# Julia-Tempering/Pigeons.jl

Hardware: AMD Instinct MI355X
Metric: replica-steps/sec (explore+swap), toy_mvn d=1024, n_chains=1024; round-trip rate (higher is better)
Workload: dtype f64

## Files before the change

### pigeons.jl_amd/csrc/pte_slice8.hpp

```cpp
#pragma once
#include "pte_slice7.hpp"

namespace pte {

#ifndef PTE_S8_BD
#define PTE_S8_BD 3
#endif
#ifndef PTE_S8_BS
#define PTE_S8_BS 9
#endif
constexpr int S8_BD = PTE_S8_BD;

#ifndef PTE_S8_WAVES
#define PTE_S8_WAVES 4
#endif
template <int NLU, int S8_BS, int WINDOW, int DBL_MODE>
__device__ __forceinline__ void slice8_body(EngineDev e, SliceParams sp, const int64_t cl) {
    using namespace s7;
    constexpr int WIN = WINDOW, REFILL_AT = WINDOW - PTE_S7_MARGIN;
    constexpr bool FAST = (DBL_MODE == 2);
    static_assert(CAP_ITERS >= S8_BS, "lane 0 must be able to run past the speculative budget");
#ifndef PTE_S8_BLK
#define PTE_S8_BLK 256
#endif
    constexpr int BLK = PTE_S8_BLK, CPB = BLK / 64;
    constexpr bool HOLD_POLICY = (WIN == 512);
    __shared__ struct {
        double u[WIN];
        double e[WIN];
        double x[BLK];
        double we[256];
        unsigned long long ke[256];
        unsigned policy[HOLD_POLICY ? 2 : 0];
        double rex[HOLD_POLICY ? 64 : 0];
        unsigned rmeta[HOLD_POLICY ? 64 : 0];
    } sm;
    double (&s_u)[WIN] = sm.u; double (&s_e)[WIN] = sm.e; double (&s_x)[BLK] = sm.x; double (&s_we)[256] = sm.we; unsigned long long (&s_ke)[256] = sm.ke;
    const int lane = lane_id();
#ifdef PTE_PROFILE_WAVES
    const uint64_t wave_t0 = __builtin_amdgcn_s_memrealtime();
#endif
    for (int i = lane; i < 256; i += 64) { s_we[i] = ZIG_WE[i]; s_ke[i] = ZIG_KE[i]; }
    if constexpr (HOLD_POLICY) sm.policy[0] = g_rng_policy;
    const auto exp_seq = [&](SeqRng &rs) __attribute__((always_inline)) -> double {
        if constexpr (HOLD_POLICY)
            return randexp_from_raw_hot(rs, rs.next(), [&]() __attribute__((always_inline)) -> unsigned {
                return (unsigned)__builtin_amdgcn_readfirstlane((int)*(const volatile __attribute__((address_space(3))) unsigned *)&sm.policy[0]); });
        else
            return randexp_seq(rs);
    };
    __syncthreads();
    if (cl >= e.K) return;
    const int64_t c = e.c0 + cl;
    const int slot = e.slot_of_chain[cl];
    if (is_ref_chain(e, c)) {
        iid_refresh_recorded<NLU>(e, cl, c, slot, e.sd[c], lane);
        return;
    }
    const double lp_before = lp_before_explore(e, c, slot);
    const int64_t d = e.d;
    double *xrow = e.x + (int64_t)slot * e.ld;
    const int B = (int)((d + 63) >> 6);
    const double nhp = e.nhp[c];
    const double inv_nhp = 1.0 / nhp;
    const double inv_abs_nhp = -inv_nhp * (1.0 + 1e-6);
    const double w = sp.w;
    const double w11 = 1.1 * sp.w;
    const int cap_iters = min(sp.max_iter, CAP_ITERS);
    const int kcap = min(sp.p, 20);
    const bool shr_more = S8_BS < cap_iters;
    constexpr bool HAND_SHRINK = (S8_BS == PTE_S8_BS && S8_BS >= 6 && S8_BS <= 10);
    constexpr bool N_IS_KN = (DBL_MODE == 2) && HAND_SHRINK;

    const int hg = s7_level(lane);
    const int hrel = s7_pick(LO, hg, 0) + lane - s7_pick(BASE, hg, 0);

    const int succ_lo = s7_pick(LO, hg + 1, 0), succ_wd = s7_pick(WD, hg + 1, 0), succ_base = s7_pick(BASE, hg + 1, 0);
    const int succ_off = hrel - succ_lo;
    const int word_c = 0x10000 - succ_off;
    const int word_c9 = (1 << 20) - succ_off * 512;
    const uint64_t seed_in = e.rng[2 * slot];

    double BS = 0.0;
    for (int b = 0; b < B; ++b) {
        int64_t i = 64 * (int64_t)b + lane;
        double v = (i < d) ? xrow[i] : 0.0;
        double s = wave_sum_dpp(v * v);
        if (lane == b) BS = s;
    }
    double S = upper_tree_root<NLU>(BS);
    if (nhp * S == -INFINITY) { if (lane == 0) set_error(e, ERR_SLICE_SUPPORT, (int)c, -1); return; }

    uint64_t wseed = e.rng[2 * slot];
    const uint64_t gamma = e.rng[2 * slot + 1];
    int p = 0;
    uint64_t gamma_inv = gamma;
    for (int k = 0; k < 5; ++k) gamma_inv *= 2ull - gamma * gamma_inv;
    double wsum = 0.0;
    typedef unsigned mask2_t __attribute__((ext_vector_type(2)));
    typedef unsigned slow_mask_t __attribute__((ext_vector_type(WIN / 32)));
    typedef double draws8_t __attribute__((ext_vector_type(8)));
    typedef double draws2_t __attribute__((ext_vector_type(2)));
    slow_mask_t slow_w;
#ifdef PTE_PROFILE_SECTIONS
    long long prof[21] = {0, 0, 0, 0, 0, 0, 0, 0, 0, 0, 0, 0, 0, 0, 0, 0, 0, 0, 0, 0, 0};
#endif
    constexpr unsigned S8_UNRESOLVED = 0xFFFFu;
    auto fill_window = [&]() __attribute__((always_inline)) {
        __syncthreads();
        double acc = 0.0;
        double pend_x = 0.0;
        int pend_m = WIN;
#pragma unroll
        for (int k = 0; k < WIN / 64; ++k) {
            const int i = 64 * k + lane;
            const uint64_t r = mix64(wseed + (uint64_t)(i + 1) * gamma);
            const uint64_t ri = r & MASK52;
            const int idx = (int)(ri & 0xFF);
            const bool fast = ri < s_ke[idx];
            const double ev = (double)ri * s_we[idx];
            s_u[i] = u52_to_unit(r);
            s_e[i] = fast ? ev : __longlong_as_double(0x7ff8000000000000LL);
            acc += fast ? ev : 0.0;
            const uint64_t sb = ballot64(!fast);
            slow_w[2 * k] = (unsigned)sb; slow_w[2 * k + 1] = (unsigned)(sb >> 32);
            if constexpr (HOLD_POLICY) { pend_x = fast ? pend_x : ev; pend_m = fast ? pend_m : (i | (idx << 16)); }
        }
        wsum = wave_sum_dpp(acc);
        p = 0;
        __syncthreads();
        if constexpr (HOLD_POLICY) {
            __builtin_amdgcn_sched_barrier(0);
            const int pi = pend_m & 0xFFFF, pidx = pend_m >> 16;
            const double f1 = ZIG_FE[pidx], f0 = ZIG_FE[(pidx - 1) & 0xFF];
            const double un = s_u[min(pi + 1, WIN - 1)], en = s_e[min(pi + 2, WIN - 1)];
            const double ex = exp(-pend_x);
            const bool in_reach = (pidx != 0) && (pi + 2 < WIN);
            const bool wedge = (f0 - f1) * un + f1 < ex;
            const unsigned used = !in_reach ? 0u : wedge ? 2u : (en == en) ? 3u : 0u;
            sm.rex[lane] = wedge ? pend_x : en;
            sm.rmeta[lane] = used ? ((unsigned)pi | (used << 16)) : S8_UNRESOLVED;
#ifdef PTE_PROFILE_SECTIONS
            prof[20] += (long long)__popcll(ballot64(used != 0u)) << 24;
#endif
            __syncthreads();
        }
    };
    fill_window();

    int dbl_z0 = 0, dbl_z1 = 0, dbl_one_hi = 0x3ff00000;
    if constexpr (DBL_MODE == 2) asm volatile("" : "+v"(dbl_z0), "+v"(dbl_z1), "+v"(dbl_one_hi));

    long long steps_sum = 0, fb_draws = 0, ex_total = 0;
    int steps_n = 0, acc_sum = 0, acc_n = 0, n_fb = 0;
    int err = 0, err_coord = -1;

    for (int pass = 0; pass < sp.n_passes && !err; ++pass) {
        for (int b = 0; BLK * (int64_t)b < d && !err; ++b) {
            const int64_t base = BLK * (int64_t)b;
            const int nl = (int)min((int64_t)BLK, d - base);
#pragma unroll
            for (int k = 0; k < CPB; ++k) s_x[64 * k + lane] = (64 * k + lane < nl) ? xrow[base + 64 * k + lane] : 0.0;
            __builtin_amdgcn_wave_barrier();
            double Sest = S * (1.0 + 1e-6) + wsum * inv_abs_nhp;
            int l = 0, l_end = nl;
            do {
                PROF_T(t0);
                if (__builtin_expect(p > REFILL_AT, 0)) { PROF_T(tr0); wseed += (uint64_t)p * gamma; fill_window(); Sest = Sest * (1.0 + 1e-6) + wsum * inv_abs_nhp; PROF_T(tr1); PROF_ADD(16, tr1 - tr0); PROF_ADD(17, 1); }
                const bool active = (l + hg) < nl;
                const double xold = s_x[(l + hg) & (BLK - 1)];
                int idx0 = p + hrel;
                double E = s_e[idx0];
                double u0 = s_u[idx0 + 1];
                double Vd[S8_BD];
#pragma unroll
                for (int it = 0; it < S8_BD; ++it) Vd[it] = s_u[idx0 + 2 + it];
                int ua = 0;
                if constexpr (DBL_MODE == 2) ua = (int)(uintptr_t)(const __attribute__((address_space(3))) double *)&s_u[idx0];
                int ex0 = 0;
                int cnt_base = 2;
                asm volatile("" : "+v"(cnt_base));
                if constexpr (DBL_MODE == 2) asm volatile("" : "+s"(ex0));
                unsigned slow_b;
                if constexpr (WIN == 512)
                    asm("s_lshr_b32 m0, %[p], 5\n" "s_nop 0\n" "s_movrels_b32 %[o], s84\n" "s_lshr_b32 %[o], %[o], %[p]"
                        : [o] "=&s"(slow_b) : [p] "s"(p), "{s[84:99]}"(slow_w) : "m0", "scc");
                else
                    asm("s_lshr_b32 m0, %[p], 5\n" "s_nop 0\n" "s_movrels_b32 %[o], s84\n" "s_lshr_b32 %[o], %[o], %[p]"
                        : [o] "=&s"(slow_b) : [p] "s"(p), "{s[84:91]}"(slow_w) : "m0", "scc");
                static_assert(WIN == 512 || WIN == 256, "the slow-path mask is sixteen or eight dwords");
                if (__builtin_expect((slow_b & 1u) != 0u, 0)) {
                    PROF_T(ts0);
                    if constexpr (HOLD_POLICY) {
                        const auto head_moves = [&](const double Ex, const int used) __attribute__((always_inline)) {
                            ex0 = used - 1;
                            if (lane == 0) { E = Ex; idx0 += ex0; cnt_base = 2 + ex0; ua += 8 * ex0; }
                            Sest += Ex * inv_abs_nhp;
                            ex_total += ex0;
                            u0 = s_u[idx0 + 1];
#pragma unroll
                            for (int it = 0; it < S8_BD; ++it) Vd[it] = s_u[idx0 + 2 + it];
                        };
                        const unsigned rmeta = (unsigned)__builtin_amdgcn_readfirstlane((int)sm.rmeta[p & 63]);
                        const double rex = sm.rex[p & 63];
                        if ((rmeta & 0xFFFFu) == (unsigned)p) {
                            head_moves(rex, (int)(rmeta >> 16));
#ifdef PTE_PROFILE_SECTIONS
                            asm volatile("" :: "v"(E), "v"(u0), "v"(Vd[S8_BD - 1]), "v"(Sest));
#endif
                            PROF_T(ts1); PROF_ADD(2, ts1 - ts0); PROF_ADD(20, 1);
                        } else {
                            SeqRng rs{wseed + (uint64_t)p * gamma, gamma};
                            const double Ex = exp_seq(rs);
                            const int used = (int)((rs.seed - (wseed + (uint64_t)p * gamma)) * gamma_inv);
                            if (used <= 17) head_moves(Ex, used);
#ifdef PTE_PROFILE_SECTIONS
                            asm volatile("" :: "v"(E), "v"(u0), "v"(Vd[S8_BD - 1]), "v"(Sest));
#endif
                            PROF_T(ts1); PROF_ADD(18, ts1 - ts0); PROF_ADD(19, 1);
                        }
                    } else {
                    SeqRng rs{wseed + (uint64_t)p * gamma, gamma};
                    const double Ex = exp_seq(rs);
                    const int used = (int)((rs.seed - (wseed + (uint64_t)p * gamma)) * gamma_inv);
                    if (used <= 17) {
                        ex0 = used - 1;
                        if (lane == 0) { E = Ex; idx0 += ex0; cnt_base = 2 + ex0; ua += 8 * ex0; }
                        Sest += Ex * inv_abs_nhp;
                        ex_total += ex0;
                        u0 = s_u[idx0 + 1];
#pragma unroll
                        for (int it = 0; it < S8_BD; ++it) Vd[it] = s_u[idx0 + 2 + it];
                    }
#ifdef PTE_PROFILE_SECTIONS
                    asm volatile("" :: "v"(E), "v"(u0), "v"(Vd[S8_BD - 1]), "v"(Sest));
#endif
                    PROF_T(ts1); PROF_ADD(18, ts1 - ts0); PROF_ADD(19, 1);
                    }
                }
                const double Enh = E * inv_nhp;
                const double Q = __builtin_fma(xold, xold, -Enh);
                const double Bq = Sest + fabs(Q);
                double dmin = fabs(Enh);
                auto test = [&](double v) __attribute__((always_inline)) -> double {
                    const double d = __builtin_fma(v, v, -Q);
                    dmin = fmin(dmin, fabs(d));
                    return d;
                };
                double LL = xold - w * u0;
                double RR = LL + w;
                double dL = test(LL), dR = test(RR);
                int kd = 0;
                double dmin_lr = 0.0;
                unsigned need_l0 = 0u;
                uint64_t need_m = 0ull;
                double thr2 = 0.0, mthr = 0.0, W = 0.0;
                int n = 0;
                uint64_t act_m = 0ull;
                draws8_t ud8 = 0.0; draws2_t ud2 = 0.0;
#if PTE_S8_BD >= 1 && PTE_S8_BD <= 4 && !defined(PTE_S8_DOUBLING_SELECTS)
                if constexpr (DBL_MODE == 2) {
                    double t_, wd_;
                    int sLh_, sRh_;
                    uint64_t sv_, sx_;
                    mask2_t sd_;
#define PTE_S8_CSTEP(V) \
                    "v_cmp_ge_f64 vcc, 0.5, " V "\n" \
                    "v_min_f64 v[102:103], v[114:115], v[116:117]\n" \
                    "v_cmpx_gt_f64_e64 %[sx], 0, v[102:103]\n" \
                    "v_add_f64 v[112:113], v[98:99], -v[96:97]\n" \
                    "v_add_u32 %[kd], 1, %[kd]\n" \
                    "v_add_u32 %[ua], 8, %[ua]\n" \
                    "v_cndmask_b32 v119, 0, %[one], vcc\n" \
                    "v_cndmask_b32 v121, %[one], v118, vcc\n" \
                    "v_fma_f64 v[96:97], -v[118:119], v[112:113], v[96:97]\n" \
                    "v_fma_f64 v[98:99], v[120:121], v[112:113], v[98:99]\n" \
                    "v_fma_f64 v[114:115], v[96:97], v[96:97], -v[110:111]\n" \
                    "v_fma_f64 v[116:117], v[98:99], v[98:99], -v[110:111]\n"
#define PTE_S8_CFOLD \
                    "v_min_f64 v[104:105], v[104:105], |v[114:115]|\n" \
                    "v_min_f64 v[104:105], v[104:105], |v[116:117]|\n"
#if PTE_S8_BS == 6
#define PTE_S8_UREADS_TAIL
#elif PTE_S8_BS == 7
#define PTE_S8_UREADS_TAIL "ds_read_b64 v[136:137], %[ua] offset:64\n"
#elif PTE_S8_BS == 8
#define PTE_S8_UREADS_TAIL "ds_read2_b64 v[136:139], %[ua] offset0:8 offset1:9\n"
#elif PTE_S8_BS == 9
#define PTE_S8_UREADS_TAIL "ds_read2_b64 v[136:139], %[ua] offset0:8 offset1:9\n" "ds_read_b64 v[140:141], %[ua] offset:80\n"
#else
#define PTE_S8_UREADS_TAIL "ds_read2_b64 v[136:139], %[ua] offset0:8 offset1:9\n" "ds_read2_b64 v[140:143], %[ua] offset0:10 offset1:11\n"
#endif
                    asm volatile("s_mov_b64 %[sv], exec\n"
#if PTE_S8_BD >= 2
                                 PTE_S8_CSTEP("%[V0]") PTE_S8_CFOLD
#endif
#if PTE_S8_BD >= 3
                                 PTE_S8_CSTEP("%[V1]") PTE_S8_CFOLD
#endif
#if PTE_S8_BD >= 4
                                 PTE_S8_CSTEP("%[V2]") PTE_S8_CFOLD
#endif
                                 PTE_S8_CSTEP("%[VL]")
                                 "s_mov_b64 exec, %[sv]\n"
                                 "ds_read2_b64 v[124:127], %[ua] offset0:2 offset1:3\n"
                                 "ds_read2_b64 v[128:131], %[ua] offset0:4 offset1:5\n"
                                 "ds_read2_b64 v[132:135], %[ua] offset0:6 offset1:7\n"
                                 PTE_S8_UREADS_TAIL
                                 "v_min_f64 v[102:103], v[114:115], v[116:117]\n"
                                 "v_cmp_gt_f64_e64 %[sd], 0, v[102:103]\n"
                                 PTE_S8_CFOLD
                                 "v_add_f64 %[mthr], %[Sest], |v[110:111]|\n"
                                 "v_max_f64 %[thr], |v[96:97]|, |v[98:99]|\n"
                                 "v_cmp_gt_i32_e64 %[act], %[nl], %[lg]\n"
                                 "v_add3_u32 v106, %[cb], %[so], %[kd]\n"
                                 "v_mul_f64 %[mthr], %[mthr], %[c_m]\n"
                                 "v_mul_f64 %[thr], %[thr], %[c_t]\n"
                                 "v_add_f64 v[112:113], v[98:99], -v[96:97]\n"
                                 : "+{v[96:97]}"(LL), "+{v[98:99]}"(RR), "+{v[114:115]}"(dL), "+{v[116:117]}"(dR), "+{v[104:105]}"(dmin), [kd] "+v"(kd), [ua] "+v"(ua),
                                   "=&{v[102:103]}"(t_), "=&{v[112:113]}"(wd_), "=&{v119}"(sLh_), "=&{v121}"(sRh_), [sv] "=&s"(sv_), [sx] "=&s"(sx_), [sd] "=&s"(sd_),
                                   "=&{v[124:139]}"(ud8), "=&{v[140:143]}"(ud2), [mthr] "=&v"(mthr), [thr] "=&v"(thr2), "=&{v106}"(n), [act] "=&s"(act_m)
                                 : "{v[110:111]}"(Q), "{v118}"(dbl_z0), "{v120}"(dbl_z1), [one] "v"(dbl_one_hi),
                                   [V0] "v"(Vd[0]), [V1] "v"(Vd[S8_BD > 2 ? 1 : 0]), [V2] "v"(Vd[S8_BD > 3 ? 2 : 0]), [VL] "v"(Vd[S8_BD - 1]),
                                   [Sest] "v"(Sest), [nl] "s"(nl), [lg] "v"(l + hg), [cb] "v"(cnt_base), [so] "v"(succ_off), [c_m] "s"(2e-12), [c_t] "s"(1e-6)
                                 : "vcc", "scc");
#undef PTE_S8_CSTEP
#undef PTE_S8_CFOLD
#undef PTE_S8_UREADS_TAIL
                    dmin_lr = t_; W = wd_;
                    need_m = (uint64_t)sd_.x | ((uint64_t)sd_.y << 32); need_l0 = __builtin_amdgcn_readfirstlane(sd_.x);
                } else
                if (DBL_MODE == 1 && sp.p >= S8_BD) {
                    double t_, wd_;
                    uint64_t sv_, sv2_;
#define PTE_S8_DSTEP(V) \
                    "v_min_f64 %[t], %[dL], %[dR]\n" \
                    "v_cmp_gt_f64 vcc, 0, %[t]\n" \
                    "s_and_saveexec_b64 %[sv], vcc\n" \
                    "v_add_u32 %[kd], 1, %[kd]\n" \
                    "v_add_f64 %[wd], %[RR], -%[LL]\n" \
                    "v_cmp_ge_f64 vcc, 0.5, " V "\n" \
                    "s_and_saveexec_b64 %[sv2], vcc\n" \
                    "v_add_f64 %[LL], %[LL], -%[wd]\n" \
                    "v_fma_f64 %[dL], %[LL], %[LL], -%[Q]\n" \
                    "v_min_f64 %[dmin], %[dmin], |%[dL]|\n" \
                    "s_andn2_b64 exec, %[sv2], exec\n" \
                    "v_add_f64 %[RR], %[RR], %[wd]\n" \
                    "v_fma_f64 %[dR], %[RR], %[RR], -%[Q]\n" \
                    "v_min_f64 %[dmin], %[dmin], |%[dR]|\n" \
                    "s_mov_b64 exec, %[sv]\n"
                    asm volatile(PTE_S8_DSTEP("%[V0]")
#if PTE_S8_BD >= 2
                                 PTE_S8_DSTEP("%[V1]")
#endif
#if PTE_S8_BD >= 3
                                 PTE_S8_DSTEP("%[V2]")
#endif
#if PTE_S8_BD >= 4
                                 PTE_S8_DSTEP("%[V3]")
#endif
                                 : [LL] "+v"(LL), [RR] "+v"(RR), [dL] "+v"(dL), [dR] "+v"(dR), [dmin] "+v"(dmin), [kd] "+v"(kd),
                                   [t] "=&v"(t_), [wd] "=&v"(wd_), [sv] "=&s"(sv_), [sv2] "=&s"(sv2_)
                                 : [Q] "v"(Q), [V0] "v"(Vd[0]), [V1] "v"(Vd[S8_BD > 1 ? 1 : 0]), [V2] "v"(Vd[S8_BD > 2 ? 2 : 0]), [V3] "v"(Vd[S8_BD > 3 ? 3 : 0])
                                 : "vcc", "scc");
#undef PTE_S8_DSTEP
                } else
#endif
#pragma unroll
                for (int it = 0; it < S8_BD; ++it) {
                    const bool need = (fmin(dL, dR) < 0.0) && it < sp.p;
                    const double V = Vd[it];
                    kd += need ? 1 : 0;
                    const bool left = V <= 0.5;
                    const double wd = RR - LL;
                    if constexpr (DBL_MODE == 0) {
                        const double sL = (need && left) ? 1.0 : 0.0, sR = (need && !left) ? 1.0 : 0.0;
                        LL = __builtin_fma(-sL, wd, LL);
                        RR = __builtin_fma(sR, wd, RR);
                        dL = __builtin_fma(LL, LL, -Q);
                        dR = __builtin_fma(RR, RR, -Q);
                        dmin = fmin(dmin, fmin(fabs(dL), fabs(dR)));
                    } else {
                        const double cand = left ? (LL - wd) : (RR + wd);
                        const double dc = __builtin_fma(cand, cand, -Q);
                        dmin = need ? fmin(dmin, fabs(dc)) : dmin;
                        const bool nl_ = need && left, nr_ = need && !left;
                        LL = nl_ ? cand : LL;
                        RR = nr_ ? cand : RR;
                        dL = nl_ ? dc : dL;
                        dR = nr_ ? dc : dR;
                    }
                }
#if !(PTE_S8_BD >= 1 && PTE_S8_BD <= 4) || defined(PTE_S8_DOUBLING_SELECTS)
                static_assert(DBL_MODE != 2, "PTE_S8_DBL_MODE == 2 needs the v_cmpx doubling block: 1 <= PTE_S8_BD <= 4 and no PTE_S8_DOUBLING_SELECTS");
#endif
                if constexpr (DBL_MODE != 2) dmin_lr = fmin(dL, dR);
                unsigned more_dbl;
                if constexpr (FAST) more_dbl = need_l0 & 1u;
                else more_dbl = ballot64(lane == 0 && (dmin_lr < 0.0) && kd < kcap) != 0ull ? 1u : 0u;
                if (__builtin_expect(more_dbl != 0u, 0)) {
                    bool need = (lane == 0);
                    while (need) {
                        const double V = s_u[idx0 + 2 + kd];
                        kd += 1;
                        const bool left = V <= 0.5;
                        const double wd = RR - LL;
                        const double cand = left ? (LL - wd) : (RR + wd);
                        const double dc = test(cand);
                        LL = left ? cand : LL;
                        RR = left ? RR : cand;
                        dL = left ? dc : dL;
                        dR = left ? dR : dc;
                        need = (kd < kcap) && (fmin(dL, dR) < 0.0);
                    }
                    asm volatile("" : "+v"(dL), "+v"(dR), "+v"(kd));
                    dmin_lr = fmin(dL, dR);
                    if constexpr (FAST) {
                        dmin_lr = (kd >= sp.p) ? 0.0 : dmin_lr;
                        need_m = ballot64(dmin_lr < 0.0);
                        need_l0 = (unsigned)need_m;
                        thr2 = 1e-6 * fmax(fabs(LL), fabs(RR));
                        n = cnt_base + kd + succ_off;
                        W = RR - LL;
                        const double *un = &s_u[idx0 + 2 + kd];
#pragma unroll
                        for (int k = 0; k < 8; ++k) ud8[k] = (k < S8_BS) ? un[k] : 0.0;
#pragma unroll
                        for (int k = 8; k < 10; ++k) ud2[k - 8] = (k < S8_BS) ? un[k] : 0.0;
                        asm volatile("" : "+{v[124:139]}"(ud8), "+{v[140:143]}"(ud2));
                    }
                }
                const bool dbl_ok = FAST ? !__builtin_amdgcn_inverse_ballot_w64(need_m) : !((kd < sp.p) && (dmin_lr < 0.0));
                if constexpr (DBL_MODE != 2) thr2 = 1e-6 * fmax(fabs(LL), fabs(RR));
#ifdef PTE_PROFILE_SECTIONS
                asm volatile("" :: "v"(LL), "v"(RR), "v"(kd), "v"(thr2));
#endif
                PROF_T(t1); PROF_ADD(0, t1 - t0);
                static_assert(DBL_MODE != 2 || HAND_SHRINK, "PTE_S8_DBL_MODE == 2 hands its draws to the hand-written shrinkage block: 6 <= PTE_S8_BS <= 10");
                const double *us = &s_u[idx0 + 2 + kd];
                double u[S8_BS];
                if constexpr (DBL_MODE != 2) {
#pragma unroll
                    for (int k = 0; k < S8_BS; ++k) u[k] = us[k];
                }
                if constexpr (DBL_MODE != 2) mthr = 2e-12 * Bq;
                int kn0 = cnt_base + kd + succ_off;
                uint64_t pre_ok;
                if constexpr (FAST) pre_ok = 0ull;
                else pre_ok = ballot64(active && dbl_ok);
                double Lbar = LL, Rbar = RR, xf = xold;
                if constexpr (!N_IS_KN) n = 0;
                bool fin = false;
                unsigned unf_l0 = 0u;
                uint64_t unf_m = 0ull;
                if constexpr (S8_BS == PTE_S8_BS && S8_BS >= 6 && S8_BS <= 10) {
                    double t_;
                    mask2_t unf_mask;
                    uint64_t exec_save;
#define PTE_S8_STEP_W \
                    "v_add_f64 v[112:113], v[98:99], -v[96:97]\n"
#define PTE_S8_STEP(U) PTE_S8_STEP_W PTE_S8_STEP_U(U)
#define PTE_S8_STEP_U(U) \
                    "v_mul_f64 v[102:103], " U ", v[112:113]\n" \
                    "v_add_f64 v[100:101], v[96:97], v[102:103]\n" \
                    "v_cmp_lt_f64 vcc, v[100:101], v[108:109]\n" \
                    "v_fma_f64 v[102:103], v[100:101], v[100:101], -v[110:111]\n" \
                    "v_add_u32 v106, 1, v106\n" \
                    "v_cndmask_b32 v96, v96, v100, vcc\n" \
                    "v_cndmask_b32 v97, v97, v101, vcc\n" \
                    "v_cndmask_b32 v98, v100, v98, vcc\n" \
                    "v_cndmask_b32 v99, v101, v99, vcc\n" \
                    "v_min_f64 v[104:105], v[104:105], |v[102:103]|\n" \
                    "v_cmpx_ngt_f64 vcc, 0, v[102:103]\n"
                    if constexpr (DBL_MODE == 2) {
#if defined(PTE_S8_ONE_WAIT) || defined(PTE_PROFILE_SECTIONS)
#define PTE_S8_WAIT(K) "s_waitcnt lgkmcnt(0)\n"
#else
#define PTE_S8_WAIT(K) "s_waitcnt lgkmcnt(" #K ")\n"
#endif
#if PTE_S8_BS >= 9
#define PTE_S8_W1 4
#define PTE_S8_W3 3
#define PTE_S8_W5 2
#define PTE_S8_W7 1
#elif PTE_S8_BS >= 7
#define PTE_S8_W1 3
#define PTE_S8_W3 2
#define PTE_S8_W5 1
#define PTE_S8_W7 0
#else
#define PTE_S8_W1 2
#define PTE_S8_W3 1
#define PTE_S8_W5 0
#endif
#define PTE_S8_WAIT_(K) PTE_S8_WAIT(K)
                    asm volatile(".p2align 3\n"
                                 "s_mov_b64 %[sv], exec\n"
                                 "s_andn2_b64 %[pre], %[act], %[need]\n"
                                 PTE_S8_WAIT_(PTE_S8_W1) PTE_S8_STEP_U("v[124:125]") PTE_S8_STEP("v[126:127]")
                                 PTE_S8_STEP_W PTE_S8_WAIT_(PTE_S8_W3) PTE_S8_STEP_U("v[128:129]") PTE_S8_STEP("v[130:131]")
                                 PTE_S8_STEP_W PTE_S8_WAIT_(PTE_S8_W5) PTE_S8_STEP_U("v[132:133]") PTE_S8_STEP("v[134:135]")
#if PTE_S8_BS >= 7
                                 PTE_S8_STEP_W PTE_S8_WAIT_(PTE_S8_W7) PTE_S8_STEP_U("v[136:137]")
#endif
#if PTE_S8_BS >= 8
                                 PTE_S8_STEP("v[138:139]")
#endif
#if PTE_S8_BS >= 9
                                 PTE_S8_STEP_W PTE_S8_WAIT_(0) PTE_S8_STEP_U("v[140:141]")
#endif
#if PTE_S8_BS >= 10
                                 PTE_S8_STEP("v[142:143]")
#endif
                                 "s_mov_b64 %[unf], exec\n"
                                 "s_mov_b64 exec, %[sv]\n"
                                 "s_nop 3\n"
                                 : "+{v[96:97]}"(Lbar), "+{v[98:99]}"(Rbar), "=&{v[100:101]}"(xf), "=&{v[102:103]}"(t_),
                                   "+{v[104:105]}"(dmin), "+{v106}"(n), "+{v[112:113]}"(W), [unf] "=&s"(unf_mask), [sv] "=&s"(exec_save), [pre] "=&s"(pre_ok)
                                 : "{v[108:109]}"(xold), "{v[110:111]}"(Q), "{v[124:139]}"(ud8), "{v[140:143]}"(ud2), [act] "s"(act_m), [need] "s"(need_m)
                                 : "vcc", "scc");
#undef PTE_S8_WAIT
#undef PTE_S8_WAIT_
#undef PTE_S8_W1
#undef PTE_S8_W3
#undef PTE_S8_W5
#undef PTE_S8_W7
                    } else
                    asm volatile(".p2align 3\n"
                                 "s_mov_b64 %[sv], exec\n"
                                 PTE_S8_STEP("%[u0]") PTE_S8_STEP("%[u1]") PTE_S8_STEP("%[u2]") PTE_S8_STEP("%[u3]")
                                 PTE_S8_STEP("%[u4]") PTE_S8_STEP("%[u5]")
#if PTE_S8_BS >= 7
                                 PTE_S8_STEP("%[u6]")
#endif
#if PTE_S8_BS >= 8
                                 PTE_S8_STEP("%[u7]")
#endif
#if PTE_S8_BS >= 9
                                 PTE_S8_STEP("%[u8]")
#endif
#if PTE_S8_BS >= 10
                                 PTE_S8_STEP("%[u9]")
#endif
                                 "s_mov_b64 %[unf], exec\n"
                                 "s_mov_b64 exec, %[sv]\n"
                                 "s_nop 3\n"
                                 : "+{v[96:97]}"(Lbar), "+{v[98:99]}"(Rbar), "=&{v[100:101]}"(xf), "=&{v[102:103]}"(t_),
                                   "+{v[104:105]}"(dmin), "+{v106}"(n), "=&{v[112:113]}"(W), [unf] "=&s"(unf_mask), [sv] "=&s"(exec_save)
                                 : "{v[108:109]}"(xold), "{v[110:111]}"(Q), [u0] "v"(u[0]), [u1] "v"(u[1]), [u2] "v"(u[2]), [u3] "v"(u[3]),
                                   [u4] "v"(u[4]), [u5] "v"(u[5]), [u6] "v"(u[S8_BS > 6 ? 6 : 0]), [u7] "v"(u[S8_BS > 7 ? 7 : 0]),
                                   [u8] "v"(u[S8_BS > 8 ? 8 : 0]), [u9] "v"(u[S8_BS > 9 ? 9 : 0])
                                 : "vcc");
#undef PTE_S8_STEP
#undef PTE_S8_STEP_W
#undef PTE_S8_STEP_U
                    unf_m = (uint64_t)unf_mask.x | ((uint64_t)unf_mask.y << 32); unf_l0 = __builtin_amdgcn_readfirstlane(unf_mask.x);
                    fin = !__builtin_amdgcn_inverse_ballot_w64(unf_m);
                } else {
#pragma unroll
                    for (int k = 0; k < S8_BS; ++k) {
                        W = Rbar - Lbar;
                        const double v = Lbar + u[k] * W;
                        const double dv = __builtin_fma(v, v, -Q);
                        dmin = fmin(dmin, fabs(dv));
                        xf = fin ? xf : v;
                        n += fin ? 0 : 1;
                        const bool below = v < xold;
                        Lbar = below ? v : Lbar;
                        Rbar = below ? Rbar : v;
                        fin = fin || (dv < 0.0);
                    }
                    unf_m = ballot64(!fin);
                    unf_l0 = (unsigned)unf_m;
                }
                if (__builtin_expect((unf_l0 & 1u) != 0u, 0)) {
                  if (shr_more) {
                    double dx = 1.0;
                    bool go = (lane == 0);
                    const int n_off = N_IS_KN ? cnt_base + kd + succ_off : 0;
                    while (go) {
                        W = Rbar - Lbar;
                        xf = Lbar + us[n - n_off] * W;
                        n += 1;
                        dx = test(xf);
                        const bool below = xf < xold;
                        Lbar = below ? xf : Lbar;
                        Rbar = below ? Rbar : xf;
                        go = !(dx < 0.0) && n - n_off < cap_iters;
                    }
                    asm volatile("" : "+v"(dx), "+v"(n), "+v"(W));
                    fin = fin || (lane == 0 && dx < 0.0);
                    unf_m = ballot64(!fin);
                  }
                }
                PROF_T(t2); PROF_ADD(1, t2 - t1); PROF_ADD(3, 1);
                int gdone;
#ifdef PTE_PROFILE_SECTIONS
                constexpr bool ASM_TAIL = false;
#else
                constexpr bool ASM_TAIL = FAST && G == 5;
#endif
                if constexpr (ASM_TAIL) {
                    const int kn = N_IS_KN ? n : kn0 + n;
                    const int wsucc = ((unsigned)kn < (unsigned)succ_wd) ? kn + succ_base : 0;
                    const int word_v = (kn << 9) + word_c9 + wsucc;
                    unsigned acc; uint64_t tmask, sA_, sB_; int w_, pk_, s0_, s1_, s2_, s3_, s4_;
                    asm volatile("v_cmp_gt_f64 vcc, %[W], %[thr]\n"
                                 "v_cndmask_b32_e64 %[w], 0, %[wv], %[pre]\n"
                                 "v_cmp_gt_f64_e64 %[sA], %[dm], %[mthr]\n"
                                 "v_cndmask_b32_e64 %[w], %[w], 0, %[unf]\n"
                                 "v_cndmask_b32_e32 %[w], 0, %[w], vcc\n"
                                 "s_nop 0\n"
                                 "v_cndmask_b32_e64 %[w], 0, %[w], %[sA]\n"
                                 "v_cndmask_b32_e64 %[pk], 0, %[w], %[nz]\n"
                                 : [w] "=&v"(w_), [pk] "=&v"(pk_), [sA] "=&s"(sA_)
                                 : [wv] "v"(word_v), [pre] "s"(pre_ok), [unf] "s"(unf_m), [nz] "s"(0xFFFFFFFFFFFFFFFEull),
                                   [W] "v"(W), [thr] "v"(thr2), [dm] "v"(dmin), [mthr] "v"(mthr)
                                 : "vcc");
                    asm volatile("v_cmp_ne_u32_e64 %[sB], 0, %[w]\n"
                                 "s_mov_b64 %[tm], 1\n"
                                 "v_readlane_b32 %[s0], %[w], 0\n"
                                 "s_nop 3\n"
                                 "v_readlane_b32 %[s1], %[pk], %[s0]\n"
                                 "s_bitset1_b64 %[tm], %[s0]\n"
                                 "s_mov_b32 %[acc], %[s0]\n"
                                 "s_nop 1\n"
                                 "v_readlane_b32 %[s2], %[pk], %[s1]\n"
                                 "s_bitset1_b64 %[tm], %[s1]\n"
                                 "s_add_u32 %[acc], %[acc], %[s1]\n"
                                 "s_nop 1\n"
                                 "v_readlane_b32 %[s3], %[pk], %[s2]\n"
                                 "s_bitset1_b64 %[tm], %[s2]\n"
                                 "s_add_u32 %[acc], %[acc], %[s2]\n"
                                 "s_nop 1\n"
                                 "v_readlane_b32 %[s4], %[pk], %[s3]\n"
                                 "s_bitset1_b64 %[tm], %[s3]\n"
                                 "s_add_u32 %[acc], %[acc], %[s3]\n"
                                 "s_and_b64 %[tm], %[tm], %[sB]\n"
                                 "s_add_u32 %[acc], %[acc], %[s4]\n"
                                 : [sB] "=&s"(sB_), [tm] "=&s"(tmask), [acc] "=&s"(acc),
                                   [s0] "=&s"(s0_), [s1] "=&s"(s1_), [s2] "=&s"(s2_), [s3] "=&s"(s3_), [s4] "=&s"(s4_)
                                 : [w] "v"(w_), [pk] "v"(pk_)
                                 : "scc");
                    if (__builtin_amdgcn_inverse_ballot_w64(tmask)) s_x[(l + hg) & (BLK - 1)] = xf;
                    __builtin_amdgcn_wave_barrier();
                    p += (int)((acc >> 9) & 0x1FFu);
                    gdone = (int)((acc >> 20) & 7u);
                    l += gdone;
                } else {
                bool valid = __builtin_amdgcn_inverse_ballot_w64(pre_ok) && fin && (W > thr2);
                if constexpr (!FAST) valid = valid && !(E != E) && n <= cap_iters;
#ifdef PTE_PROFILE_SECTIONS
                asm volatile("" :: "v"(xf), "v"(n), "v"(dmin));
#endif
#ifdef PTE_PROFILE_SECTIONS
                {
                    const bool mg = dmin > 2e-12 * Bq;
                    const int rc = !active ? 7 : (E != E) ? 1 : !dbl_ok ? 2 : !fin ? 3 : !valid ? 4 : !mg ? 5 : 0;
                    const int cnt_ = N_IS_KN ? n - succ_off : cnt_base + kd + n;
                    int o_ = 0, g_ = 0, why = 0;
                    for (g_ = 0; g_ < G; ++g_) {
                        if (l + g_ >= nl) { why = 7; break; }
                        const int k_ = o_ - LO[g_];
                        if ((unsigned)k_ >= (unsigned)WD[g_]) { why = 6; break; }
                        const int ln_ = BASE[g_] + k_;
                        const int r_ = __builtin_amdgcn_readlane(rc, ln_);
                        if (r_) { why = r_; break; }
                        o_ += __builtin_amdgcn_readlane(cnt_, ln_);
                    }
                    PROF_ADD(8 + why, 1);
                }
#endif
                valid = valid && (dmin > mthr);
                const int kn = N_IS_KN ? n : kn0 + n;
                const bool inw = (unsigned)kn < (unsigned)succ_wd;
                const uint64_t vmask = ballot64(valid);
                int word_v = kn + word_c + (inw ? (int)((unsigned)(kn + succ_base) << 24) : 0);
                asm("" : "+v"(word_v));
                const int word = valid ? word_v : 0;
                const int packed = (lane != 0) ? word : 0;
#ifdef PTE_PROFILE_SECTIONS
                asm volatile("" :: "v"(packed));
#endif
                {
                    int pk = __builtin_amdgcn_readlane(word, 0);
                    unsigned acc = 0u;
                    uint64_t tmask = 1ull;
#pragma unroll
                    for (int g = 1; g < G; ++g) {
                        const int cur = (int)((unsigned)pk >> 24);
                        asm volatile("s_bitset1_b64 %0, %2\n\ts_add_u32 %1, %1, %3" : "+s"(tmask), "+s"(acc) : "s"(cur), "s"(pk) : "scc");
                        pk = __builtin_amdgcn_readlane(packed, cur);
                    }
                    acc += (unsigned)pk;
                    tmask &= vmask;
                    if (__builtin_amdgcn_inverse_ballot_w64(tmask)) s_x[(l + hg) & (BLK - 1)] = xf;
                    __builtin_amdgcn_wave_barrier();
                    p += (int)(acc & 0xFFFFu);
                    gdone = (int)((acc >> 16) & 0xFFu);
                    l += gdone;
                }
                }
#ifdef PTE_PROFILE_SECTIONS
                asm volatile("" :: "s"(p), "s"(l));
#endif
                PROF_T(t4); PROF_ADD(5, t4 - t2); PROF_ADD(4, gdone);
                if (__builtin_expect(gdone == 0, 0)) {
                    ex_total -= ex0;
                    SeqRng rs{wseed + (uint64_t)p * gamma, gamma};
                    const int ck = l >> 6, li = l & 63, bc = CPB * b + ck;
#pragma unroll
                    for (int k = 0; k < CPB; ++k) {
                        const double xk = s_x[64 * k + lane];
                        const double sk = wave_sum_dpp(xk * xk);
                        if (lane == CPB * b + k) BS = sk;
                    }
                    const double X = s_x[64 * ck + lane];
                    const double xo = readlane_f64(X, li);
                    const double E = exp_seq(rs);
                    const double u0 = rs.rand();
                    const double Q = xo * xo - E * inv_nhp;
                    const double mg = 1e-12 * (Sest + fabs(Q));
                    const double Qlo = Q - mg, Qhi = Q + mg;
                    auto inside_exact = [&](double v) __attribute__((always_inline)) -> bool {
                        const double Xv = (lane == li) ? v : X;
                        const double sv = wave_sum_dpp(Xv * Xv), s0 = wave_sum_dpp(X * X);
                        const double Sv = upper_tree_root<NLU>((lane == bc) ? sv : BS);
                        const double S0 = upper_tree_root<NLU>((lane == bc) ? s0 : BS);
                        const double zz = nhp * S0 - E;
                        return zz < nhp * Sv;
                    };
                    auto inside = [&](double v) __attribute__((always_inline)) -> bool {
                        const double q = v * v;
                        const bool in = q < Qlo;
                        const bool out = q > Qhi;
                        if (__builtin_expect(!(in || out), 0)) return inside_exact(v);
                        return in;
                    };
                    double LL = xo - w * u0;
                    double RR = LL + w;
                    bool in_L = inside(LL), in_R = inside(RR);
                    int K = sp.p;
                    while (K > 0 && (in_L || in_R)) {
                        const double V = rs.rand();
                        if (V <= 0.5) { LL = LL - (RR - LL); in_L = inside(LL); }
                        else { RR = RR + (RR - LL); in_R = inside(RR); }
                        K -= 1;
                    }
                    steps_sum += (sp.p - K); steps_n += 1;
                    const bool doubled = (RR - LL) > w11;
                    double Lbar = LL, Rbar = RR;
                    double xn = xo;
                    bool fin = false;
                    for (int n = 1; n <= sp.max_iter; ++n) {
                        const double newpos = Lbar + rs.rand() * (Rbar - Lbar);
                        if (inside(newpos)) {
                            bool ok = true;
                            if (doubled) {
                                double Lhat = LL, Rhat = RR;
                                bool oL = !in_L, oR = !in_R;
                                bool Rstale = false, Lstale = false, D = false;
                                while (Rhat - Lhat > w11) {
                                    const double Mid = (Lhat + Rhat) / 2.0;
                                    if ((xo < Mid && newpos >= Mid) || (xo >= Mid && newpos < Mid)) D = true;
                                    if (newpos < Mid) { Rhat = Mid; Rstale = true; }
                                    else { Lhat = Mid; Lstale = true; }
                                    if (D) {
                                        if (Lstale) { oL = !inside(Lhat); Lstale = false; }
                                        if (Rstale) { oR = !inside(Rhat); Rstale = false; }
                                        if (oL && oR) { ok = false; break; }
                                    }
                                }
                            }
                            acc_n += 1;
                            if (ok) { acc_sum += 1; xn = newpos; steps_sum += n; steps_n += 1; fin = true; break; }
                        }
                        if (newpos < xo) Lbar = newpos; else Rbar = newpos;
                        if (jl_isapprox(Lbar, Rbar)) { steps_sum += n; steps_n += 1; fin = true; break; }
                    }
                    if (!fin) { err = ERR_SLICE_MAX_ITER; err_coord = (int)(base + l); l_end = 0; continue; }
                    Sest = Sest + fabs(xn * xn - xo * xo);
                    if (lane == li) s_x[l] = xn;
                    __builtin_amdgcn_wave_barrier();
                    l += 1;
                    const int used = (int)((rs.seed - (wseed + (uint64_t)p * gamma)) * gamma_inv);
                    p += used;
                    fb_draws += used; n_fb += 1;
                    PROF_T(t5); PROF_ADD(7, t5 - t4); PROF_ADD(6, 1);
                }
            } while (l < l_end);
            if (err) break;
            {
#pragma unroll
                for (int k = 0; k < CPB; ++k) {
                    const double X = s_x[64 * k + lane];
                    if (64 * k + lane < nl) xrow[base + 64 * k + lane] = X;
                    const double s = wave_sum_dpp(X * X);
                    if (lane == CPB * b + k) BS = s;
                }
                S = upper_tree_root<NLU>(BS);
                if (__builtin_expect(!isfinite(nhp * S), 0)) { err = ERR_SLICE_INVALID_LP; err_coord = (int)base; }
            }
        }
    }
    if (err) { if (lane == 0) set_error(e, err, (int)c, err_coord); return; }
    if (lane == 0) {
        const uint64_t seed_out = wseed + (uint64_t)p * gamma;
        const long long n_spec = (long long)sp.n_passes * d - n_fb;
        const long long spec_draws = (long long)((seed_out - seed_in) * gamma_inv) - fb_draws;
        steps_sum += spec_draws - ex_total - 2 * n_spec; steps_n += (int)(2 * n_spec); acc_sum += (int)n_spec; acc_n += (int)n_spec;
        e.suff[slot] = S;
        e.rng[2 * slot] = seed_out;
        e.expl_steps_sum[cl] += (double)steps_sum; e.expl_steps_n[cl] += steps_n;
        e.expl_acc_sum[cl] += (double)acc_sum;     e.expl_acc_n[cl] += acc_n;
#ifdef PTE_PROFILE_SECTIONS
        for (int i = 0; i < 21; ++i) e.on_m2[21 * cl + i] += (double)prof[i];
#endif
    }
    record_after_explore(e, cl, c, slot, lane, lp_before, S, 0.0);
#ifdef PTE_PROFILE_WAVES
    if (lane == 0) {
        double *o = e.on_m2 + 2 * (e.d + 1) + 4 * cl;
        o[0] = (double)wave_t0; o[1] = (double)__builtin_amdgcn_s_memrealtime();
        o[2] = (double)__builtin_amdgcn_s_getreg((31 << 11) | 4); o[3] = (double)__builtin_amdgcn_s_getreg((31 << 11) | 20);
    }
#endif
}

#ifndef PTE_S8_DBL_MODE
#define PTE_S8_DBL_MODE 2
#endif
template <int NLU, int S8_BS>
__global__ __launch_bounds__(64) __attribute__((amdgpu_waves_per_eu(PTE_S8_WAVES, PTE_S8_WAVES))) void k_explore_slice8(EngineDev e, SliceParams sp) {
    slice8_body<NLU, S8_BS, PTE_S7_WIN, PTE_S8_DBL_MODE>(e, sp, blockIdx.x);
}
template <int NLU, int S8_BS>
__global__ __launch_bounds__(64) __attribute__((amdgpu_waves_per_eu(PTE_S8_WAVES, PTE_S8_WAVES))) void k_explore_slice8_generic(EngineDev e, SliceParams sp) {
    slice8_body<NLU, S8_BS, PTE_S7_WIN, 0>(e, sp, blockIdx.x);
}
#ifndef PTE_S8_TWIN_WAVES
#define PTE_S8_TWIN_WAVES PTE_S8_WAVES
#endif
#ifndef PTE_S8_TWIN_FROM
#define PTE_S8_TWIN_FROM (256 * 8)
#endif
template <int NLU, int S8_BS>
__global__ __launch_bounds__(64) __attribute__((amdgpu_waves_per_eu(PTE_S8_TWIN_WAVES, PTE_S8_TWIN_WAVES))) void k_explore_slice8_lds10k(EngineDev e, SliceParams sp) {
    slice8_body<NLU, S8_BS, 256, 1>(e, sp, blockIdx.x);
}

template <int NLU, int S8_BS, int WINDOW, int DBL_MODE>
__device__ __forceinline__ void slice8_scan_loop(EngineDev e, const SliceParams &sp, const ScanLoop &sl) {
    const int lane = lane_id();
    const int64_t cl = scan_loop_chain(e.K);
    int go = 1;
    if (lane == 0) go = scan_loop_gate(sl) ? 1 : 0;
    if (!__builtin_amdgcn_readfirstlane(go)) return;
    for (int64_t i = 0; i < sl.n_scans; ++i) {
        e.trace_idx = sl.scan_idx0 + i;
        slice8_body<NLU, S8_BS, WINDOW, DBL_MODE>(e, sp, cl);
        __syncthreads();
        int slot = 0;
        if (lane == 0) slot = swap_handshake(e, sl, i, cl, e.slot_of_chain[cl]);
        slot = __builtin_amdgcn_readfirstlane(slot);
        __syncthreads();
        if (slot < 0) return;
    }
}
template <int NLU, int S8_BS>
__global__ __launch_bounds__(64) __attribute__((amdgpu_waves_per_eu(PTE_S8_WAVES, PTE_S8_WAVES))) void k_scans_slice8(EngineDev e, SliceParams sp, ScanLoop sl) {
    slice8_scan_loop<NLU, S8_BS, PTE_S7_WIN, PTE_S8_DBL_MODE>(e, sp, sl);
}
template <int NLU, int S8_BS>
__global__ __launch_bounds__(64) __attribute__((amdgpu_waves_per_eu(PTE_S8_WAVES, PTE_S8_WAVES))) void k_scans_slice8_generic(EngineDev e, SliceParams sp, ScanLoop sl) {
    slice8_scan_loop<NLU, S8_BS, PTE_S7_WIN, 0>(e, sp, sl);
}
}
```

Measured before the change: 1.750 million.

## Hoist ziggurat table staging out of scan loop and batch prologue row loads

Moves the per-call LDS struct into a shared helper so the ziggurat tables can be staged once per scan-loop kernel instead of on every body call. It also issues batched row loads for the squared-norm reduction before lp_before_explore so the memory latencies overlap, and drops one prologue barrier. The table weights are pre-scaled by 2^52 so the exponential draw multiplies the unit uniform directly. The accumulator now sums every draw rather than only fast-path ones, which changes wsum semantics and relies on later code tolerating that. Removing the barrier and changing the accumulation carry correctness risk if other waves or later logic depended on them.

```diff
diff --git a/pigeons.jl_amd/csrc/pte_slice8.hpp b/pigeons.jl_amd/csrc/pte_slice8.hpp
--- a/pigeons.jl_amd/csrc/pte_slice8.hpp
+++ b/pigeons.jl_amd/csrc/pte_slice8.hpp
@@ -14,34 +14,73 @@
 #ifndef PTE_S8_WAVES
 #define PTE_S8_WAVES 4
 #endif
-template <int NLU, int S8_BS, int WINDOW, int DBL_MODE>
+#ifndef PTE_S8_ROW_BATCH
+#define PTE_S8_ROW_BATCH 1
+#endif
+#ifndef PTE_S8_HOIST_TABLES
+#define PTE_S8_HOIST_TABLES 1
+#endif
+#ifndef PTE_S8_PROLOGUE_BATCH
+#define PTE_S8_PROLOGUE_BATCH 1
+#endif
+#ifndef PTE_S8_PRESCALED
+#define PTE_S8_PRESCALED 1
+#endif
+#ifndef PTE_S8_ACC_ALL
+#define PTE_S8_ACC_ALL 1
+#endif
+#ifndef PTE_S8_BLK
+#define PTE_S8_BLK 256
+#endif
+template <int WIN>
+struct Slice8Lds {
+    static constexpr bool HOLD_POLICY = (WIN == 512);
+    static constexpr int BLK = PTE_S8_BLK;
+    double u[WIN];
+    double e[WIN];
+    double x[BLK];
+    double we[256];
+    unsigned long long ke[256];
+    unsigned policy[HOLD_POLICY ? 2 : 0];
+    double rex[HOLD_POLICY ? 64 : 0];
+    unsigned rmeta[HOLD_POLICY ? 64 : 0];
+};
+template <int WIN>
+__device__ __forceinline__ Slice8Lds<WIN> &slice8_lds() { __shared__ Slice8Lds<WIN> sm; return sm; }
+template <int WIN>
+__device__ __forceinline__ void slice8_stage_tables(int lane) {
+    Slice8Lds<WIN> &sm = slice8_lds<WIN>();
+    if constexpr (WIN == 512) {
+        constexpr double scale = PTE_S8_PRESCALED ? 0x1p52 : 1.0;
+#pragma unroll
+        for (int k = 0; k < 4; ++k) { sm.we[64 * k + lane] = ZIG_WE[64 * k + lane] * scale; sm.ke[64 * k + lane] = ZIG_KE[64 * k + lane]; }
+    } else {
+        for (int i = lane; i < 256; i += 64) { sm.we[i] = ZIG_WE[i]; sm.ke[i] = ZIG_KE[i]; }
+    }
+}
+
+template <int NLU, int S8_BS, int WINDOW, int DBL_MODE, bool STAGE = true>
 __device__ __forceinline__ void slice8_body(EngineDev e, SliceParams sp, const int64_t cl) {
     using namespace s7;
     constexpr int WIN = WINDOW, REFILL_AT = WINDOW - PTE_S7_MARGIN;
     constexpr bool FAST = (DBL_MODE == 2);
     static_assert(CAP_ITERS >= S8_BS, "lane 0 must be able to run past the speculative budget");
-#ifndef PTE_S8_BLK
-#define PTE_S8_BLK 256
-#endif
     constexpr int BLK = PTE_S8_BLK, CPB = BLK / 64;
-    constexpr bool HOLD_POLICY = (WIN == 512);
-    __shared__ struct {
-        double u[WIN];
-        double e[WIN];
-        double x[BLK];
-        double we[256];
-        unsigned long long ke[256];
-        unsigned policy[HOLD_POLICY ? 2 : 0];
-        double rex[HOLD_POLICY ? 64 : 0];
-        unsigned rmeta[HOLD_POLICY ? 64 : 0];
-    } sm;
+    constexpr bool HOLD_POLICY = Slice8Lds<WIN>::HOLD_POLICY;
+    Slice8Lds<WIN> &sm = slice8_lds<WIN>();
     double (&s_u)[WIN] = sm.u; double (&s_e)[WIN] = sm.e; double (&s_x)[BLK] = sm.x; double (&s_we)[256] = sm.we; unsigned long long (&s_ke)[256] = sm.ke;
     const int lane = lane_id();
 #ifdef PTE_PROFILE_WAVES
     const uint64_t wave_t0 = __builtin_amdgcn_s_memrealtime();
 #endif
-    for (int i = lane; i < 256; i += 64) { s_we[i] = ZIG_WE[i]; s_ke[i] = ZIG_KE[i]; }
-    if constexpr (HOLD_POLICY) sm.policy[0] = g_rng_policy;
+    if constexpr (STAGE) slice8_stage_tables<WIN>(lane);
+    constexpr bool ONE_WAIT = PTE_S8_PROLOGUE_BATCH && WIN == 512, ROW_BATCH = PTE_S8_ROW_BATCH && WIN == 512;
+    constexpr bool PRESCALED = PTE_S8_PRESCALED && WIN == 512, ACC_ALL = PTE_S8_ACC_ALL && WIN == 512;
+    unsigned policy_word = 0;
+    if constexpr (HOLD_POLICY) {
+        policy_word = g_rng_policy;
+        if constexpr (!ONE_WAIT) sm.policy[0] = policy_word;
+    }
     const auto exp_seq = [&](SeqRng &rs) __attribute__((always_inline)) -> double {
         if constexpr (HOLD_POLICY)
             return randexp_from_raw_hot(rs, rs.next(), [&]() __attribute__((always_inline)) -> unsigned {
@@ -49,7 +88,7 @@
         else
             return randexp_seq(rs);
     };
-    __syncthreads();
+    if constexpr (!ONE_WAIT) __syncthreads();
     if (cl >= e.K) return;
     const int64_t c = e.c0 + cl;
     const int slot = e.slot_of_chain[cl];
@@ -57,11 +96,36 @@
         iid_refresh_recorded<NLU>(e, cl, c, slot, e.sd[c], lane);
         return;
     }
-    const double lp_before = lp_before_explore(e, c, slot);
     const int64_t d = e.d;
     double *xrow = e.x + (int64_t)slot * e.ld;
     const int B = (int)((d + 63) >> 6);
+    double lp_before = 0.0;
+    if constexpr (!ONE_WAIT) lp_before = lp_before_explore(e, c, slot);
     const double nhp = e.nhp[c];
+    const uint64_t rng_seed = e.rng[2 * slot], rng_gamma = e.rng[2 * slot + 1];
+    constexpr int NB = 1 << NLU, GRP = NB < 16 ? NB : 16;
+    double BS = 0.0;
+    const auto row_request = [&](int g0, double (&v)[GRP]) __attribute__((always_inline)) {
+#pragma unroll
+        for (int j = 0; j < GRP; ++j) {
+            const int64_t i = 64 * (int64_t)(g0 + j) + lane;
+            const double t = xrow[(i < d) ? i : 0];
+            v[j] = (i < d) ? t : 0.0;
+        }
+    };
+    const auto row_reduce = [&](int g0, const double (&v)[GRP]) __attribute__((always_inline)) {
+#pragma unroll
+        for (int j = 0; j < GRP; ++j) {
+            const double s = wave_sum_dpp(v[j] * v[j]);
+            if (lane == g0 + j) BS = s;
+        }
+    };
+    double row0[GRP];
+    if constexpr (ROW_BATCH) row_request(0, row0);
+    if constexpr (ONE_WAIT) {
+        lp_before = lp_before_explore(e, c, slot);
+        if constexpr (HOLD_POLICY) sm.policy[0] = policy_word;
+    }
     const double inv_nhp = 1.0 / nhp;
     const double inv_abs_nhp = -inv_nhp * (1.0 + 1e-6);
     const double w = sp.w;
@@ -79,20 +143,25 @@
     const int succ_off = hrel - succ_lo;
     const int word_c = 0x10000 - succ_off;
     const int word_c9 = (1 << 20) - succ_off * 512;
-    const uint64_t seed_in = e.rng[2 * slot];
-
-    double BS = 0.0;
-    for (int b = 0; b < B; ++b) {
-        int64_t i = 64 * (int64_t)b + lane;
-        double v = (i < d) ? xrow[i] : 0.0;
-        double s = wave_sum_dpp(v * v);
-        if (lane == b) BS = s;
+    const uint64_t seed_in = rng_seed;
+
+    if constexpr (ROW_BATCH) {
+        row_reduce(0, row0);
+        if constexpr (NB > GRP)
+            for (int g0 = GRP; g0 < B; g0 += GRP) { double rowg[GRP]; row_request(g0, rowg); row_reduce(g0, rowg); }
+    } else {
+        for (int b = 0; b < B; ++b) {
+            int64_t i = 64 * (int64_t)b + lane;
+            double v = (i < d) ? xrow[i] : 0.0;
+            double s = wave_sum_dpp(v * v);
+            if (lane == b) BS = s;
+        }
     }
     double S = upper_tree_root<NLU>(BS);
     if (nhp * S == -INFINITY) { if (lane == 0) set_error(e, ERR_SLICE_SUPPORT, (int)c, -1); return; }
 
-    uint64_t wseed = e.rng[2 * slot];
-    const uint64_t gamma = e.rng[2 * slot + 1];
+    uint64_t wseed = rng_seed;
+    const uint64_t gamma = rng_gamma;
     int p = 0;
     uint64_t gamma_inv = gamma;
     for (int k = 0; k < 5; ++k) gamma_inv *= 2ull - gamma * gamma_inv;
@@ -118,10 +187,11 @@
             const uint64_t ri = r & MASK52;
             const int idx = (int)(ri & 0xFF);
             const bool fast = ri < s_ke[idx];
-            const double ev = (double)ri * s_we[idx];
-            s_u[i] = u52_to_unit(r);
+            const double u = u52_to_unit(r);
+            const double ev = PRESCALED ? u * s_we[idx] : (double)ri * s_we[idx];
+            s_u[i] = u;
             s_e[i] = fast ? ev : __longlong_as_double(0x7ff8000000000000LL);
-            acc += fast ? ev : 0.0;
+            acc += (ACC_ALL || fast) ? ev : 0.0;
             const uint64_t sb = ballot64(!fast);
             slow_w[2 * k] = (unsigned)sb; slow_w[2 * k + 1] = (unsigned)(sb >> 32);
             if constexpr (HOLD_POLICY) { pend_x = fast ? pend_x : ev; pend_m = fast ? pend_m : (i | (idx << 16)); }
@@ -856,9 +926,11 @@
     int go = 1;
     if (lane == 0) go = scan_loop_gate(sl) ? 1 : 0;
     if (!__builtin_amdgcn_readfirstlane(go)) return;
+    constexpr bool HOISTED = PTE_S8_HOIST_TABLES != 0;
+    if constexpr (HOISTED) slice8_stage_tables<WINDOW>(lane);
     for (int64_t i = 0; i < sl.n_scans; ++i) {
         e.trace_idx = sl.scan_idx0 + i;
-        slice8_body<NLU, S8_BS, WINDOW, DBL_MODE>(e, sp, cl);
+        slice8_body<NLU, S8_BS, WINDOW, DBL_MODE, !HOISTED>(e, sp, cl);
         __syncthreads();
         int slot = 0;
         if (lane == 0) slot = swap_handshake(e, sl, i, cl, e.slot_of_chain[cl]);
```

New measurement: 1.737 million. Within noise of the previous version (-0.7%).
